# genjax-community/genjax

Hardware: AMD Instinct MI355X
Metric: particle_steps_per_sec (higher is better)
Workload: dtype f32; 1 GPU; gmm_c8_d16 ImportanceK: propagate+reweight+LSE, systematic resample, gather (BASELINE.json configs[1]); k_particles_per_gpu=1048576, k_particles_total=1048576, rng_stream=flat, exchange=none

## Files before the change

### genjax_amd/csrc/gjx_run.hip

```cpp
#include <hip/hip_ext.h>

#include "gjx_device.h"
#include "gjx_host.h"
#include "gjx_scan.h"
#include "gjx_tile.h"

#include <string.h>
#include <type_traits>

namespace gjx {

struct RunArgs {
  const gjx_site* sites;
  const float* tab;
  int n_sites, n_slots;
  key2 key;
  int64_t K, offset;
  float* choices;
  float* score;
  float* weight;
  float* logw;
  const float* logw_in;
  const float* sub;
  float* site_scores;
// ... 224 lines not shown
    else {
      score += lp;
      if (given) weight += lp;
    }
    if (a.site_scores && active) {
      float* ss = a.site_scores + (int64_t)j * K + i;
      *ss = inst == 0 ? lp : *ss + lp;
    }
    }
    }
    j0 += m;
  }
  float lw = weight;
  if (a.logw_in) lw += a.logw_in[ii];
  if (a.sub) lw -= a.sub[ii];
  if (active) {
    if (a.score) a.score[i] = score;
    if (a.weight) a.weight[i] = weight;
    if (a.logw) a.logw[i] = lw;
  }
  if (a.partials) {
    float bm, bsum;
    block_lse_partial<256>(lw, active, red, bm, bsum);
    if (a.lse) lse_publish_and_finish<256>(bm, bsum, a.partials, a.ticket, (int)gridDim.x, a.log_k_total, a.lse, red);
    else if (threadIdx.x == 0) a.partials[blockIdx.x] = pack_f2(bm, bsum);
  }
}

struct GmmArgs {
  const float* tab;
  int C;
  int logits_off, mu_off, sig_off;
  int r_off, r_len, y_off;
  key2 key;
  int64_t K, offset;
  float* choices;
  float* score;
  float* weight;
  float* logw;
  const float* logw_in;
  const float* sub;
  unsigned long long* partials;
  unsigned* ticket;
  float* lse;
  float log_k_total;
  const float* aux;
  double u;
  float* rows_out;
  int32_t* ancestors;
  unsigned long long* agg;
  unsigned* ctrl;
  unsigned long long* timeline;
  unsigned long long* tile_S;
  int32_t* tile_E;
};

template <int PPT>
struct VecStore;
template <>
struct VecStore<1> {
  static GJX_DEV void st(float* p, const float (&v)[1]) { *p = v[0]; }
};
template <>
struct VecStore<2> {
  static GJX_DEV void st(float* p, const float (&v)[2]) { *reinterpret_cast<float2*>(p) = make_float2(v[0], v[1]); }
};
template <>
struct VecStore<4> {
  static GJX_DEV void st(float* p, const float (&v)[4]) {
    *reinterpret_cast<float4*>(p) = make_float4(v[0], v[1], v[2], v[3]);
  }
};

typedef unsigned u32x4 __attribute__((ext_vector_type(4)));
constexpr int kAuxSc1 = 16;
GJX_DEV __amdgpu_buffer_rsrc_t buffer_of(const void* base, uint32_t bytes) {
  return __builtin_amdgcn_make_buffer_rsrc(const_cast<void*>(base), 0, (int)bytes, 0x00020000);
}
GJX_DEV void store4_sc1(__amdgpu_buffer_rsrc_t rs, uint32_t lane_off, uint32_t row_off, const float (&v)[4]) {
  const u32x4 x = {__float_as_uint(v[0]), __float_as_uint(v[1]), __float_as_uint(v[2]), __float_as_uint(v[3])};
  __builtin_amdgcn_raw_buffer_store_b128(x, rs, (int)lane_off, (int)row_off, kAuxSc1);
  asm volatile("s_nop 1");
}
GJX_DEV float load_sc1(__amdgpu_buffer_rsrc_t rs, uint32_t lane_off, uint32_t row_off) {
  return __uint_as_float(__builtin_amdgcn_raw_buffer_load_b32(rs, (int)lane_off, (int)row_off, kAuxSc1));
}
GJX_DEV int32_t load_sc1(const int32_t* p) { return __hip_atomic_load(p, __ATOMIC_RELAXED, __HIP_MEMORY_SCOPE_AGENT); }

template <int RNG, int D, int PPT, int THREADS>
__global__ __launch_bounds__(THREADS) void k_run_gmm(GmmArgs a) {
  constexpr int DS = D + 4;
  extern __shared__ __attribute__((aligned(16))) float smem[];
  const int C = a.C;
  float* s_mu = smem;
  float* s_sig = s_mu + C * DS;
  float* s_logit = s_sig + C * DS;
  float* s_race = s_logit + C;
  float* s_zlp = s_race + C;
  float* s_cdf = s_zlp + C;
  float* s_y = s_cdf + C;
  float* s_rr = s_y + D;
  float* s_misc = s_rr + D;
  const float* __restrict__ tab = a.tab;

  float* s_lsig = s_misc + 32;
  float* s_lr = s_lsig + C * DS;
  for (int t = threadIdx.x; t < C * D; t += THREADS) {
    const int c = t / D, d = t % D;
    const float sg = tab[a.sig_off + t];
    s_mu[c * DS + d] = tab[a.mu_off + t];
    s_sig[c * DS + d] = sg;
    s_lsig[c * DS + d] = fast_log(sg);
  }
  for (int t = threadIdx.x; t < D; t += THREADS) {
    const float r = tab[a.r_off + (a.r_len == 1 ? 0 : t)];
    s_y[t] = tab[a.y_off + t];
    s_rr[t] = fast_rcp(r);
    s_lr[t] = fast_log(r);
  }
  for (int t = threadIdx.x; t < C; t += THREADS) {
    const float l = tab[a.logits_off + t];
    s_logit[t] = l;
    s_race[t] = kLn2 * fast_exp(-l);
  }
  __syncthreads();
  if (threadIdx.x < 64) {
    float mx = -INFINITY;
    for (int c = threadIdx.x; c < C; c += 64) mx = fmaxf(mx, s_logit[c]);
    mx = wave_max(mx);
    float se = 0.0f;
    for (int c = threadIdx.x; c < C; c += 64) se += fast_exp(s_logit[c] - mx);
    se = wave_sum(se);
    const float lse = mx + fast_log(se);
    for (int c = threadIdx.x; c < C; c += 64) {
      float sl = 0.0f;
      for (int d = 0; d < D; ++d) sl += s_lsig[c * DS + d];
      s_zlp[c] = (s_logit[c] - lse) - sl - (float)D * kHalfLog2Pi;
    }
    if (threadIdx.x == 63) {
      float sl = 0.0f;
      for (int d = 0; d < D; ++d) sl += s_lr[d];
      s_misc[0] = -sl - (float)D * kHalfLog2Pi;
    }
    if (threadIdx.x == 0) {
      float run = 0.0f;
      for (int c = 0; c < C; ++c) { run += fast_exp(s_logit[c] - mx); s_cdf[c] = run; }
    }
  }
  __syncthreads();

  const int64_t K = a.K;
  const int64_t tile = (int64_t)THREADS * PPT;
  const int64_t ntiles = (K + tile - 1) / tile;
  const uint64_t goff = (uint64_t)a.offset;
  const key2 fkey = (RNG == GJX_RNG_FLAT && (goff >> 32)) ? threefry2x32(a.key, 0xFFFFFFFFu, (uint32_t)(goff >> 32)) : a.key;
  float tmax = -INFINITY;
  float tsum = 0.0f;
  for (int64_t tix = blockIdx.x; tix < ntiles; tix += gridDim.x) {
    const int64_t i0 = tix * tile + (int64_t)threadIdx.x * PPT;
    bool act[PPT];
    uint32_t c0[PPT];
    key2 sk1[PPT], sk2[PPT];
#pragma unroll
    for (int p = 0; p < PPT; ++p) {
      act[p] = (i0 + p) < K;
      const uint64_t gi = goff + (uint64_t)(act[p] ? i0 + p : K - 1);
// ... 44 lines not shown
        if (RNG == GJX_RNG_JAX32) {
          const key2 h0 = threefry2x32(sk2[p], 0u, (uint32_t)d0);
          b0 = h0.a ^ h0.b;
          if (d0 + 1 < D) { const key2 h1 = threefry2x32(sk2[p], 0u, (uint32_t)(d0 + 1)); b1 = h1.a ^ h1.b; }
        } else {
          const key2 h = threefry2x32(fkey, c0[p], (2u << GJX_FLAT_SITE_SHIFT) | (uint32_t)(d0 >> 1));
          b0 = h.a; b1 = h.b;
        }
        const int zo = z[p] * DS + d0;
        float n0, n1;
        if (RNG == GJX_RNG_FLAT) box_muller(b0, b1, n0, n1);
        else { n0 = normal_from_bits_fast(b0); n1 = (d0 + 1 < D) ? normal_from_bits_fast(b1) : 0.0f; }
        {
          const float x = fmaf(s_sig[zo], n0, s_mu[zo]);
          qx[p] = fmaf(n0, n0, qx[p]);
          const float zy = (s_y[d0] - x) * s_rr[d0];
          qy[p] = fmaf(zy, zy, qy[p]);
          xa[p] = x;
        }
        if (d0 + 1 < D) {
          const float x = fmaf(s_sig[zo + 1], n1, s_mu[zo + 1]);
          qx[p] = fmaf(n1, n1, qx[p]);
          const float zy = (s_y[d0 + 1] - x) * s_rr[d0 + 1];
          qy[p] = fmaf(zy, zy, qy[p]);
          xb[p] = x;
        } else xb[p] = 0.0f;
      }
      float* r0 = ch + (int64_t)(1 + d0) * K + i0;
      if (full) {
        VecStore<PPT>::st(r0, xa);
        if (d0 + 1 < D) VecStore<PPT>::st(r0 + K, xb);
      } else {
#pragma unroll
        for (int p = 0; p < PPT; ++p) if (act[p]) { r0[p] = xa[p]; if (d0 + 1 < D) r0[K + p] = xb[p]; }
      }
    }
    float sc[PPT], wt[PPT], lw[PPT];
#pragma unroll
    for (int p = 0; p < PPT; ++p) {
      wt[p] = fmaf(-0.5f, qy[p], s_misc[0]);
      sc[p] = fmaf(-0.5f, qx[p], s_zlp[z[p]]) + wt[p];
      float l = wt[p];
      const int64_t ii = act[p] ? i0 + p : K - 1;
      if (a.logw_in) l += a.logw_in[ii];
      if (a.sub) l -= a.sub[ii];
      lw[p] = l;
    }
    if (full) {
      if (a.score) VecStore<PPT>::st(a.score + i0, sc);
      if (a.weight) VecStore<PPT>::st(a.weight + i0, wt);
      if (a.logw) VecStore<PPT>::st(a.logw + i0, lw);
    } else {
#pragma unroll
      for (int p = 0; p < PPT; ++p) if (act[p]) {
        if (a.score) a.score[i0 + p] = sc[p];
        if (a.weight) a.weight[i0 + p] = wt[p];
        if (a.logw) a.logw[i0 + p] = lw[p];
      }
    }
#pragma unroll
    for (int p = 0; p < PPT; ++p) if (act[p]) {
      const float nm = fmaxf(tmax, lw[p]);
      if (nm > -INFINITY) tsum = tsum * fast_exp(tmax - nm) + fast_exp(lw[p] - nm);
      tmax = nm;
    }
  }
  if (a.partials) {
    constexpr int NW = THREADS / 64;
    float* red = s_misc + 8;
    const int lane = threadIdx.x & 63, wid = threadIdx.x >> 6;
    const float wm = wave_max(tmax);
    const float ws = wave_sum(wm > -INFINITY ? tsum * fast_exp(tmax - wm) : 0.0f);
    if (lane == 0) { red[wid] = wm; red[NW + wid] = ws; }
    __syncthreads();
    float bm = red[0];
    for (int w = 1; w < NW; ++w) bm = fmaxf(bm, red[w]);
    float bsum = 0.0f;
    for (int w = 0; w < NW; ++w) bsum += bm > -INFINITY ? red[NW + w] * fast_exp(red[w] - bm) : 0.0f;
    if (a.lse) lse_publish_and_finish<THREADS>(bm, bsum, a.partials, a.ticket, (int)gridDim.x, a.log_k_total, a.lse, red);
    else if (threadIdx.x == 0) a.partials[blockIdx.x] = pack_f2(bm, bsum);
  }
}

__host__ __device__ inline int gmm_aux_floats(int C, int D) { return C * (4 * D + 4) + 2 * C + 8; }

__global__ __launch_bounds__(256) void k_gmm_prepare(GmmArgs a, int D, float* aux) {
  const int C = a.C, RS = 4 * D + 4;
  const float* __restrict__ tab = a.tab;
  float* s_t = aux; float* s_zlp = s_t + C * RS; float* s_cdf = s_zlp + C; float* s_misc = s_cdf + C;
  for (int t = threadIdx.x; t < C * (D + 1); t += 256) {
    const int c = t / (D + 1), d = t % (D + 1);
    float mu = 0.0f, sg = 0.0f, av = 0.0f, bv = 0.0f;
    if (d < D) {
      mu = tab[a.mu_off + c * D + d];
      sg = tab[a.sig_off + c * D + d];
      const float rr = fast_rcp(tab[a.r_off + (a.r_len == 1 ? 0 : d)]);
      av = (tab[a.y_off + d] - mu) * rr;
      bv = sg * rr;
    }
    float* q = s_t + c * RS + 4 * d;
    q[0] = mu; q[1] = sg; q[2] = av; q[3] = bv;
  }
  if (threadIdx.x < 64) {
    float mx = -INFINITY;
    for (int c = threadIdx.x; c < C; c += 64) mx = fmaxf(mx, tab[a.logits_off + c]);
    mx = wave_max(mx);
    float se = 0.0f;
    for (int c = threadIdx.x; c < C; c += 64) se += fast_exp(tab[a.logits_off + c] - mx);
    se = wave_sum(se);
    const float lse = mx + fast_log(se);
    for (int c = threadIdx.x; c < C; c += 64) {
      float sl = 0.0f;
      for (int d = 0; d < D; ++d) sl += fast_log(tab[a.sig_off + c * D + d]);
      s_zlp[c] = (tab[a.logits_off + c] - lse) - sl - (float)D * kHalfLog2Pi;
    }
    if (threadIdx.x == 63) {
      float sl = 0.0f;
      for (int d = 0; d < D; ++d) sl += fast_log(tab[a.r_off + (a.r_len == 1 ? 0 : d)]);
      s_misc[0] = -sl - (float)D * kHalfLog2Pi;
      for (int j = 1; j < 8; ++j) s_misc[j] = 0.0f;
    }
    if (threadIdx.x == 0) {
      float run = 0.0f;
      for (int c = 0; c < C; ++c) { run += fast_exp(tab[a.logits_off + c] - mx); s_cdf[c] = run; }
    }
  }
}

template <int D, int PPT, int THREADS, bool STEP = false, bool TILES = false>
__global__ __launch_bounds__(THREADS) void k_run_gmm_flat(GmmArgs a) {
  static_assert(!STEP || (PPT == 4 && THREADS == 256), "the one-launch step works on tiles of 256 x 4 particles");
  static_assert(!TILES || (PPT == 4 && THREADS == 256 && !STEP), "tile totals: a block's tile is one quantisation tile of 1024 particles");
  __shared__ float red_tm[4];
  __shared__ uint64_t red_tq[4];
  constexpr int RS = 4 * D + 4;
  constexpr int NPAIR = (D + 1) / 2;
  unsigned epoch = 0;
  unsigned long long tag = 0;
  if (STEP && a.timeline && threadIdx.x == 0) a.timeline[blockIdx.x * 8] = __builtin_amdgcn_s_memrealtime();
  if (STEP) tag = grid_tag(a.ctrl, &epoch);
  const __amdgpu_buffer_rsrc_t rs_ch = buffer_of(a.choices, STEP ? (uint32_t)((1 + D) * a.K * 4) : 0u);
  constexpr int NHASH = (9 + 23 * (D == 1 ? 2 : D) + 63) / 64;
  constexpr bool UNROLLED = D <= 16;
  extern __shared__ __attribute__((aligned(16))) float smem[];
  const int C = a.C;
  float* s_t = smem; float* s_zlp = s_t + C * RS; float* s_cdf = s_zlp + C; float* s_misc = s_cdf + C;
  const int64_t K = a.K;
  const int64_t tile = (int64_t)THREADS * PPT;
  const int64_t ntiles = (K + tile - 1) / tile;
  const uint64_t goff = (uint64_t)a.offset;
  const key2 fkey = (goff >> 32) ? threefry2x32(a.key, 0xFFFFFFFFu, (uint32_t)(goff >> 32)) : a.key;

  const int naux = gmm_aux_floats(C, D);
  constexpr int NPRE = 4;
  float pre[NPRE];
#pragma unroll
  for (int j = 0; j < NPRE; ++j) {
    const int t = threadIdx.x + j * THREADS;
    pre[j] = t < naux ? a.aux[t] : 0.0f;
  }
  int64_t tix = blockIdx.x;
  uint32_t hz[PPT];
  auto cat_bits = [&](int64_t t) {
#pragma unroll
    for (int p = 0; p < PPT; ++p) {
      int64_t i = t * tile + (int64_t)threadIdx.x * PPT + p;
      i = i < K ? i : K - 1;
      hz[p] = threefry2x32(fkey, (uint32_t)(goff + (uint64_t)i), (1u << GJX_FLAT_SITE_SHIFT)).a;
    }
  };
  if (tix < ntiles) cat_bits(tix);
#pragma unroll
  for (int j = 0; j < NPRE; ++j) {
    const int t = threadIdx.x + j * THREADS;
    if (t < naux) smem[t] = pre[j];
  }
  for (int t = threadIdx.x + NPRE * THREADS; t < naux; t += THREADS) smem[t] = a.aux[t];
  __syncthreads();

  float tmax = -INFINITY;
  float tsum = 0.0f;
  float lw_tile[PPT];
#pragma unroll
  for (int p = 0; p < PPT; ++p) lw_tile[p] = -INFINITY;
  const float cdf_total = s_cdf[C - 1];
  for (; tix < ntiles; tix += gridDim.x) {
    const int64_t i0 = tix * tile + (int64_t)threadIdx.x * PPT;
    if (i0 >= K) break;
    uint32_t c0[PPT];
#pragma unroll
    for (int p = 0; p < PPT; ++p) c0[p] = (uint32_t)(goff + (uint64_t)(i0 + p));
    int z[PPT];
    float zf[PPT], target[PPT];
    uint32_t neg[PPT];
#pragma unroll
    for (int p = 0; p < PPT; ++p) {
      target[p] = (__uint_as_float(__builtin_amdgcn_alignbit(0x7Fu, hz[p], 9)) - 1.0f) * cdf_total;
      neg[p] = 0u;
    }
    for (int c = 0; c < C - 1; ++c) {
      const float cd = s_cdf[c];
#pragma unroll
      for (int p = 0; p < PPT; ++p) neg[p] += __float_as_uint(target[p] - cd) >> 31;
    }
#pragma unroll
    for (int p = 0; p < PPT; ++p) { z[p] = (C - 1) - (int)neg[p]; zf[p] = (float)z[p]; }
    float* ch = a.choices;
    if constexpr (STEP) store4_sc1(rs_ch, (uint32_t)i0 * 4u, 0u, zf); else VecStore<PPT>::st(ch + i0, zf);
    float qx[PPT], qy[PPT];
#pragma unroll
    for (int p = 0; p < PPT; ++p) { qx[p] = 0.0f; qy[p] = 0.0f; }
    uint32_t w[PPT][UNROLLED ? 2 * NHASH : 2];
    BitStreamRT<GJX_RNG_FLAT> bs[UNROLLED ? 1 : PPT];
    if (!UNROLLED) {
#pragma unroll
      for (int p = 0; p < PPT; ++p) { bs[p].key = fkey; bs[p].c0 = c0[p]; bs[p].site_hi = 2u << GJX_FLAT_SITE_SHIFT; bs[p].h0 = bs[p].h1 = 0xFFFFFFFFu; }
    }
    constexpr int UF = UNROLLED ? NPAIR : 1;
#pragma unroll UF
    for (int k = 0; k < NPAIR; ++k) {
      const int d0 = 2 * k;
      float xa[PPT], xb[PPT];
#pragma unroll
      for (int p = 0; p < PPT; ++p) {
        uint32_t wa, wb;
        if constexpr (UNROLLED) {
          const int last = D == 1 ? 1 : 2 * k + 1;
          const int need = (((23 * last) >> 5) + ((((23 * last) & 31) != 0) ? 1 : 0)) >> 1;
          const int prev_last = 2 * (k - 1) + 1;
          const int have = k == 0 ? -1 : ((((23 * prev_last) >> 5) + ((((23 * prev_last) & 31) != 0) ? 1 : 0)) >> 1);
#pragma unroll
          for (int h = 0; h < NHASH; ++h) if (h > have && h <= need) {
            const key2 hh = threefry2x32(fkey, c0[p], (2u << GJX_FLAT_SITE_SHIFT) | (uint32_t)h);
            w[p][2 * h] = hh.a; w[p][2 * h + 1] = hh.b;
          }
          wa = GJX_FIELD(w[p], 2 * k);
          wb = GJX_FIELD(w[p], 2 * k + 1);
        } else {
          wa = bs[p].get((uint32_t)d0);
          wb = bs[p].get((uint32_t)d0 + 1u);
        }
        const float u1 = 2.0f - __uint_as_float(__builtin_amdgcn_alignbit(0x7Fu, wa, 9));
        const float rsq = __builtin_amdgcn_logf(u1) * (-2.0f * kLn2);
        const float r = fast_sqrt(rsq);
        const float4* row = reinterpret_cast<const float4*>(s_t + z[p] * RS) + d0;
        if (D == 1) {
          const float u2 = __uint_as_float(__builtin_amdgcn_alignbit(0x7Fu, wb, 9));
          const float n0 = r * __builtin_amdgcn_cosf(u2);
          const float4 t0 = row[0];
          const float x = fmaf(t0.y, n0, t0.x);
          qx[p] = fmaf(n0, n0, qx[p]);
          const float zy = fmaf(-t0.w, n0, t0.z);
          qy[p] = fmaf(zy, zy, qy[p]);
          xa[p] = x; xb[p] = 0.0f;
        } else {
          const float u2 = __uint_as_float(__builtin_amdgcn_alignbit(0x7Fu, wb, 9));
          const float n0 = r * __builtin_amdgcn_cosf(u2), n1 = r * __builtin_amdgcn_sinf(u2);
          const float4 t0 = row[0], t1 = row[1];
          xa[p] = fmaf(t0.y, n0, t0.x);
          xb[p] = fmaf(t1.y, n1, t1.x);
          qx[p] += rsq;
          const float zy0 = fmaf(-t0.w, n0, t0.z), zy1 = fmaf(-t1.w, n1, t1.z);
          qy[p] = fmaf(zy0, zy0, qy[p]);
          qy[p] = fmaf(zy1, zy1, qy[p]);
        }
      }
      float* r0 = ch + (int64_t)(1 + d0) * K + i0;
      if constexpr (STEP) {
        store4_sc1(rs_ch, (uint32_t)i0 * 4u, (uint32_t)(1 + d0) * (uint32_t)K * 4u, xa);
        if (D > 1) store4_sc1(rs_ch, (uint32_t)i0 * 4u, (uint32_t)(2 + d0) * (uint32_t)K * 4u, xb);
      }
      else { VecStore<PPT>::st(r0, xa); if (D > 1) VecStore<PPT>::st(r0 + K, xb); }
#pragma unroll
      for (int p = 0; p < PPT; ++p) asm volatile("" : "+v"(qx[p]), "+v"(qy[p]));
      __builtin_amdgcn_sched_barrier(0);
    }
    float sc[PPT], wt[PPT], lw[PPT];
    const float wconst = s_misc[0];
#pragma unroll
    for (int p = 0; p < PPT; ++p) {
      wt[p] = fmaf(-0.5f, qy[p], wconst);
      sc[p] = fmaf(-0.5f, qx[p], s_zlp[z[p]]) + wt[p];
      float l = wt[p];
      if (a.logw_in) l += a.logw_in[i0 + p];
      if (a.sub) l -= a.sub[i0 + p];
      lw[p] = l;
    }
    if (a.score) VecStore<PPT>::st(a.score + i0, sc);
    if (a.weight) VecStore<PPT>::st(a.weight + i0, wt);
    if (a.logw) VecStore<PPT>::st(a.logw + i0, lw);
    if (STEP) {
#pragma unroll
      for (int p = 0; p < PPT; ++p) lw_tile[p] = lw[p];
    }
    float m4 = tmax;
#pragma unroll
    for (int p = 0; p < PPT; ++p) m4 = fmaxf(m4, lw[p]);
    if (m4 > -INFINITY) {
      float s4 = tsum * fast_exp(tmax - m4);
#pragma unroll
      for (int p = 0; p < PPT; ++p) s4 += fast_exp(lw[p] - m4);
      tsum = s4;
    }
    tmax = m4;
    if constexpr (TILES) {
      uint64_t q[PPT], inc;
      const int e = tile_quantise<THREADS, PPT>(lw, red_tm, red_tq, q, inc);
      if (threadIdx.x == 0) {
        const uint64_t tot = sum_partials<THREADS / 64>(red_tq);
        a.tile_S[tix] = tot;
        a.tile_E[tix] = tot ? e : kTileDead;
      }
    }
    if (tix + gridDim.x < ntiles) cat_bits(tix + gridDim.x);
  }
  constexpr int NW = THREADS / 64;
  __shared__ float red[2 * NW + 2];
  float bm = -INFINITY, bsum = 0.0f;
  if (a.partials || STEP) {
    const int lane = threadIdx.x & 63, wid = threadIdx.x >> 6;
    const float wm = wave_max(tmax);
    const float ws = wave_sum(wm > -INFINITY ? tsum * fast_exp(tmax - wm) : 0.0f);
    if (lane == 0) { red[wid] = wm; red[NW + wid] = ws; }
    __syncthreads();
    bm = red[0];
    for (int w2 = 1; w2 < NW; ++w2) bm = fmaxf(bm, red[w2]);
    for (int w2 = 0; w2 < NW; ++w2) bsum += bm > -INFINITY ? red[NW + w2] * fast_exp(red[w2] - bm) : 0.0f;
  }
  if constexpr (!STEP) {
    if (a.partials) {
      if (a.lse) lse_publish_and_finish<THREADS>(bm, bsum, a.partials, a.ticket, (int)gridDim.x, a.log_k_total, a.lse, red);
      else if (threadIdx.x == 0) a.partials[blockIdx.x] = pack_f2(bm, bsum);
    }
  } else {
    __shared__ ScanSmem sm;
#define GJX_STAMP(n) do { if (a.timeline && threadIdx.x == 0) a.timeline[blockIdx.x * 8 + (n)] = __builtin_amdgcn_s_memrealtime(); } while (0)
    GJX_STAMP(1);
    unsigned long long* aggA0 = a.agg;
    unsigned long long* aggA1 = aggA0 + gridDim.x;
    unsigned long long* aggB = aggA1 + gridDim.x;
    unsigned long long* aggC = aggB + gridDim.x;
    const int64_t i0 = (int64_t)blockIdx.x * tile + (int64_t)threadIdx.x * PPT;
    if (threadIdx.x == 0) {
      grid_publish(aggA0, tag, (unsigned long long)__float_as_uint(bm));
      grid_publish(aggA1, tag, (unsigned long long)__float_as_uint(bsum));
    }
    float gmax = -INFINITY, gsum = 0.0f;
    {
      float pm[8];
      int np = 0;
      grid_gather(aggA0, tag, a.ctrl, [&](int, unsigned long long v) { pm[np++] = __uint_as_float((uint32_t)v); });
      np = 0;
      grid_gather(aggA1, tag, a.ctrl, [&](int, unsigned long long v) {
        const float px = pm[np++], py = __uint_as_float((uint32_t)v);
        const float nm = fmaxf(gmax, px);
        if (nm > -INFINITY) gsum = gsum * fast_exp(gmax - nm) + py * fast_exp(px - nm);
        gmax = nm;
      });
    }
    {
      const float wm = wave_max(gmax);
      const float ws = wave_sum(wm > -INFINITY ? gsum * fast_exp(gmax - wm) : 0.0f);
      __syncthreads();
      if ((threadIdx.x & 63) == 0) { red[threadIdx.x >> 6] = wm; red[NW + (threadIdx.x >> 6)] = ws; }
      __syncthreads();
      gmax = fmaxf(fmaxf(red[0], red[1]), fmaxf(red[2], red[3]));
      gsum = 0.0f;
      for (int w2 = 0; w2 < 4; ++w2) gsum += gmax > -INFINITY ? red[NW + w2] * fast_exp(red[w2] - gmax) : 0.0f;
    }
    if (a.lse && blockIdx.x == 0 && threadIdx.x == 0) {
      const float l = gmax > -INFINITY ? gmax + logf(gsum) : -INFINITY;
      a.lse[0] = gmax; a.lse[1] = gsum; a.lse[2] = l; a.lse[3] = l - a.log_k_total;
    }
    GJX_STAMP(2);
    tile_scan_expand<PPT, true>(lw_tile, 1, gmax, i0, K, a.u, K, a.ancestors, nullptr, nullptr, aggB, tag, a.ctrl, epoch, false, sm);
    GJX_STAMP(3);
    asm volatile("s_waitcnt vmcnt(0)" ::: "memory");
    __syncthreads();
    if (threadIdx.x == 0) grid_publish(aggC, tag, 1ull);
    grid_gather(aggC, tag, a.ctrl, [&](int, unsigned long long) {});
    __syncthreads();
    if (blockIdx.x == 0 && threadIdx.x == 0)
      __hip_atomic_store(&a.ctrl[0], epoch + 1u, __ATOMIC_RELAXED, __HIP_MEMORY_SCOPE_AGENT);
    GJX_STAMP(4);
    int32_t an[PPT];
#pragma unroll
    for (int p = 0; p < PPT; ++p) an[p] = load_sc1(a.ancestors + i0 + p);
    constexpr int R = 1 + D;
#pragma unroll 4
    for (int r = 0; r < R; ++r) {
      float v[PPT];
#pragma unroll
      for (int p = 0; p < PPT; ++p) v[p] = load_sc1(rs_ch, (uint32_t)an[p] * 4u, (uint32_t)r * (uint32_t)K * 4u);
      VecStore<PPT>::st(a.rows_out + (int64_t)r * K + i0, v);
    }
    asm volatile("s_waitcnt vmcnt(0)" ::: "memory");
    GJX_STAMP(5);
#undef GJX_STAMP
  }
}

__global__ __launch_bounds__(256) void k_lse_finish(const float2* partials, int n, float log_k_total, float* out) {
  __shared__ float red[8];
  float m = -INFINITY;
  for (int t = threadIdx.x; t < n; t += 256) m = fmaxf(m, partials[t].x);
  m = wave_max(m);
  if ((threadIdx.x & 63) == 0) red[threadIdx.x >> 6] = m;
  __syncthreads();
  const float bm = fmaxf(fmaxf(red[0], red[1]), fmaxf(red[2], red[3]));
  float s = 0.0f;
  for (int t = threadIdx.x; t < n; t += 256) {
    const float2 p = partials[t];
    if (p.x > -INFINITY) s += p.y * fast_exp(p.x - bm);
  }
  s = wave_sum(s);
  if ((threadIdx.x & 63) == 0) red[4 + (threadIdx.x >> 6)] = s;
  __syncthreads();
  if (threadIdx.x == 0) {
    const float bs = red[4] + red[5] + red[6] + red[7];
    const float lse = bm > -INFINITY ? bm + logf(bs) : -INFINITY;
    out[0] = bm; out[1] = bs; out[2] = lse; out[3] = lse - log_k_total;
  }
}

__global__ __launch_bounds__(256) void k_lse_partial(const float* x, int64_t K, float2* partials) {
// ... 99 lines not shown
void fill_gmm_args(GmmArgs& a, const gjx_program* prog, const GmmShape& g) {
  a.tab = prog->tab_dev; a.C = g.C;
  a.logits_off = g.logits_off; a.mu_off = g.mu_off; a.sig_off = g.sig_off;
  a.r_off = g.r_off; a.r_len = g.r_len; a.y_off = g.y_off;
  a.aux = prog->aux_dev;
}

bool gmm_usable(const gjx_program* p, GmmShape* g) {
  if (env_int("GJX_FORCE_GENERIC", 0) || !match_gmm(p, g)) return false;
  if (p->rng_mode == GJX_RNG_JAX32) return true;
  return p->aux_dev != nullptr && p->n_aux >= gmm_aux_floats(g->C, g->D);
}

}

int gjx_launch_lse_finish(const void* partials, int n, int64_t K_total, float* out, hipStream_t st) {
  hipLaunchKernelGGL(k_lse_finish, dim3(1), dim3(256), 0, st, (const float2*)partials, n,
                     (float)log((double)K_total), out);
  GJX_CHECK_LAUNCH("lse_finish");
  return GJX_OK;
}

extern "C" int gjx_event_create(void** ev) {
  if (!ev) return gjx_fail(GJX_EINVAL, "gjx_event_create: bad argument");
  hipEvent_t e;
  const hipError_t r = hipEventCreate(&e);
  if (r != hipSuccess) return gjx_fail_hip(r, "gjx_event_create");
  *ev = (void*)e;
  return GJX_OK;
}
extern "C" int gjx_event_destroy(void* ev) {
  if (ev) (void)hipEventDestroy((hipEvent_t)ev);
  return GJX_OK;
}
extern "C" int gjx_event_elapsed_us(void* start, void* stop, float* us) {
  if (!start || !stop || !us) return gjx_fail(GJX_EINVAL, "gjx_event_elapsed_us: bad argument");
  hipError_t r = hipEventSynchronize((hipEvent_t)stop);
  if (r != hipSuccess) return gjx_fail_hip(r, "gjx_event_elapsed_us");
  float ms = 0.0f;
  r = hipEventElapsedTime(&ms, (hipEvent_t)start, (hipEvent_t)stop);
  if (r != hipSuccess) return gjx_fail_hip(r, "gjx_event_elapsed_us");
  *us = ms * 1000.0f;
  return GJX_OK;
}


extern "C" int gjx_program_aux_floats(const gjx_program* prog) {
  if (!prog || !prog->sites) return GJX_EINVAL;
  GmmShape g;
  if (prog->rng_mode == GJX_RNG_FLAT && match_gmm(prog, &g)) return gmm_aux_floats(g.C, g.D);
  return 0;
}

extern "C" int gjx_program_prepare(const gjx_program* prog, float* aux_dev, int32_t n_aux, void* stream) {
  if (!prog || !prog->sites || !prog->tab_dev) return gjx_fail(GJX_EINVAL, "gjx_program_prepare: null program");
  const int need = gjx_program_aux_floats(prog);
  if (need <= 0) return GJX_OK;
  if (!aux_dev || n_aux < need) return gjx_fail(GJX_EINVAL, "gjx_program_prepare: aux buffer too small (gjx_program_aux_floats)");
  GmmShape g;
  match_gmm(prog, &g);
  GmmArgs a = {};
  fill_gmm_args(a, prog, g);
  hipLaunchKernelGGL(k_gmm_prepare, dim3(1), dim3(256), 0, (hipStream_t)stream, a, g.D, aux_dev);
  GJX_CHECK_LAUNCH("gjx_program_prepare");
  return GJX_OK;
}

struct EnginePlan {
  int engine, ppt, grid;
  GmmShape g;
};

static EnginePlan plan_engine(const gjx_program* prog, int64_t K, int64_t particle_offset, bool want_site_scores, bool want_tiles = false) {
  EnginePlan e;
  e.engine = ENGINE_GENERIC; e.ppt = 1; e.grid = (int)((K + 255) / 256);
  const char* env = getenv("GJX_ENGINE");
  const bool interp = env_int("GJX_FORCE_GENERIC", 0) || (env && !strcmp(env, "interp"));
  if (interp) return e;
  const bool gen_first = env && !strcmp(env, "gen");
  const bool same_hi = ((uint64_t)particle_offset >> 32) == ((uint64_t)(particle_offset + K - 1) >> 32);
  bool has_proposal = false;
  for (int j = 0; j < prog->n_sites; ++j) has_proposal = has_proposal || (prog->sites[j].flags & GJX_SITE_PROPOSAL) || prog->sites[j].mode == GJX_MODE_OBS_PROPOSED;
  auto try_gmm = [&]() {
    if (has_proposal || want_site_scores || !same_hi || !gmm_usable(prog, &e.g)) return false;
    int ppt = env_int("GJX_GMM_PPT", 4);
    if (ppt != 1 && ppt != 2 && ppt != 4) ppt = 4;
    if (K % ppt != 0) ppt = 1;
    const int64_t tile = 256 * (int64_t)ppt, ntiles = (K + tile - 1) / tile;
    const int maxgrid = env_int("GJX_GMM_GRID", 2048);
    e.engine = ENGINE_GMM; e.ppt = ppt; e.grid = (int)(ntiles < maxgrid ? ntiles : maxgrid);
    return true;
  };
  auto try_gen = [&]() {
    if (env_int("GJX_NO_CODEGEN", 0) || !same_hi) return false;
    const int ppt = gen_pick_ppt(prog, K, want_tiles && K % 1024 == 0);
    RunVariant gv;
    if (!decode(ppt, &gv) || gen_available(prog, ppt) != GJX_OK) return false;
    const int64_t tile = gv.particles_per_block(), ntiles = (K + tile - 1) / tile;
    static const int resident = [] { int dev = 0, cus = 256; (void)hipGetDevice(&dev); (void)hipDeviceGetAttribute(&cus, hipDeviceAttributeMultiprocessorCount, dev); return 4 * (cus > 0 ? cus : 256); }();
    int maxgrid = env_int("GJX_GEN_GRID", gv.mfma ? (1 << 20) : (gv.wide ? 2 * resident : resident));
    if (gv.wide && maxgrid > (int)((K + 255) / 256) && maxgrid > 4096) maxgrid = (int)((K + 255) / 256) > 4096 ? (int)((K + 255) / 256) : 4096;
    e.engine = ENGINE_GEN; e.ppt = ppt; e.grid = (int)(ntiles < maxgrid ? ntiles : maxgrid);
    return true;
  };
  if (gen_first) { if (!try_gen()) try_gmm(); }
  else if (!try_gmm()) try_gen();
  return e;
}

extern "C" int gjx_program_engine(const gjx_program* prog) {
  if (!prog || !prog->sites) return GJX_EINVAL;
  return plan_engine(prog, 1024, 0, false).engine;
}

extern "C" int gjx_run_partials_count(const gjx_program* prog, int64_t K, int64_t particle_offset) {
  if (!prog || !prog->sites || K <= 0) return GJX_EINVAL;
  return plan_engine(prog, K, particle_offset, false).grid;
}

extern "C" int gjx_run_program(const gjx_program* prog, uint32_t key0, uint32_t key1, int64_t K,
                               int64_t particle_offset, float* choices, float* score, float* weight,
                               float* logw, const float* logw_in, const float* sub,
                               float* site_scores, float* lse, int64_t K_total, void* workspace,
                               size_t workspace_bytes, void* stream) {
  gjx_run_opts o;
  memset(&o, 0, sizeof(o));
  return gjx_run_program_ex(prog, key0, key1, K, particle_offset, choices, score, weight, logw, logw_in, sub, site_scores, lse, K_total,
                            workspace, workspace_bytes, stream, &o, nullptr);
}

extern "C" int gjx_run_program_ex(const gjx_program* prog, uint32_t key0, uint32_t key1, int64_t K,
                                  int64_t particle_offset, float* choices, float* score, float* weight,
                                  float* logw, const float* logw_in, const float* sub,
                                  float* site_scores, float* lse, int64_t K_total, void* workspace,
                                  size_t workspace_bytes, void* stream, const gjx_run_opts* opts, gjx_run_info* info_out) {
  gjx_run_opts no_opts;
  memset(&no_opts, 0, sizeof(no_opts));
  const gjx_run_opts& op = opts ? *opts : no_opts;
  gjx_run_info info = {0, 0, 0};
  hipEvent_t ev0 = nullptr, ev1 = nullptr;
  if (op.flags & GJX_RUN_TIME_DISPATCH) { ev0 = (hipEvent_t)op.start_event; ev1 = (hipEvent_t)op.stop_event; }
  if (info_out) *info_out = info;
  if (!prog || !prog->sites || !prog->sites_dev || !prog->tab_dev) return gjx_fail(GJX_EINVAL, "gjx_run_program: null program");
  if (K < 0 || prog->n_sites < 0) return gjx_fail(GJX_EINVAL, "gjx_run_program: negative size");
  if (K == 0) return GJX_OK;
  if (prog->n_slots > 0 && !choices) return gjx_fail(GJX_EINVAL, "gjx_run_program: choices is null");
  if (lse && !logw) return gjx_fail(GJX_EINVAL, "gjx_run_program: lse needs logw");
  if (prog->rng_mode == GJX_RNG_FLAT) {
    int plain = 0, local = 0, tag = 0;
    for (int j = 0; j < prog->n_sites; ++j) {
      const int sc = prog->sites[j].scan;
      if (sc == 0) { ++plain; tag = 0; }
      else { if (sc != tag) { tag = sc; local = 0; } ++local; }
      if (plain > GJX_FLAT_MAX_SITES || local > GJX_FLAT_MAX_SITES)
        return gjx_fail(GJX_EUNSUPPORTED, "gjx_run_program: FLAT stream supports at most 1023 sites per Scan step and 1023 outside Scans");
    }
  }
  for (int j = 0; j < prog->n_sites; ++j) {
    const gjx_site& sj = prog->sites[j];
    if (sj.mode != GJX_MODE_OBS_MASK) continue;
    if (sj.kind == GJX_DIRICHLET) return gjx_fail(GJX_EUNSUPPORTED, "gjx_run_program: a dirichlet site cannot be masked per particle");
    if (sj.slot < 0 || sj.obs_off < 0 || sj.obs_off >= prog->n_slots) return gjx_fail(GJX_EINVAL, "gjx_run_program: OBS_MASK needs a value slot and a flag slot");
  }
  hipStream_t st = (hipStream_t)stream;
  unsigned long long* partials = nullptr;
  unsigned* ticket = nullptr;
  if (lse || (workspace && logw)) {
// ... 179 lines not shown
```

Measured before the change: 18.72 billion particle-steps/s.

## Use 32-bit indexing, buffer loads/stores, and popcount CDF search in flat GMM kernel

Converts the flat GMM kernel's particle indexing from 64-bit to 32-bit arithmetic, capping K on the host so the narrower math stays valid. Global loads and stores of choices, scores, weights and aux go through per-tile buffer resources. The categorical CDF search packs comparison sign bits 32 at a time and counts them with popcount. The aim is to cut address arithmetic and per-comparison ALU work. The cost is more per-tile descriptor setup and reliance on buffer-descriptor bounds behaviour.

```diff
diff --git a/genjax_amd/csrc/gjx_run.hip b/genjax_amd/csrc/gjx_run.hip
--- a/genjax_amd/csrc/gjx_run.hip
+++ b/genjax_amd/csrc/gjx_run.hip
@@ -330,6 +330,45 @@
   __builtin_amdgcn_raw_buffer_store_b128(x, rs, (int)lane_off, (int)row_off, kAuxSc1);
   asm volatile("s_nop 1");
 }
+template <int PPT>
+struct BufStore;
+template <>
+struct BufStore<1> {
+  static GJX_DEV void st(__amdgpu_buffer_rsrc_t rs, uint32_t lane_off, const float (&v)[1]) {
+    __builtin_amdgcn_raw_buffer_store_b32(__float_as_uint(v[0]), rs, (int)lane_off, 0, 0);
+  }
+};
+template <>
+struct BufStore<2> {
+  static GJX_DEV void st(__amdgpu_buffer_rsrc_t rs, uint32_t lane_off, const float (&v)[2]) {
+    typedef unsigned u32x2 __attribute__((ext_vector_type(2)));
+    const u32x2 x = {__float_as_uint(v[0]), __float_as_uint(v[1])};
+    __builtin_amdgcn_raw_buffer_store_b64(x, rs, (int)lane_off, 0, 0);
+  }
+};
+template <>
+struct BufStore<4> {
+  static GJX_DEV void st(__amdgpu_buffer_rsrc_t rs, uint32_t lane_off, const float (&v)[4]) {
+    const u32x4 x = {__float_as_uint(v[0]), __float_as_uint(v[1]), __float_as_uint(v[2]), __float_as_uint(v[3])};
+    __builtin_amdgcn_raw_buffer_store_b128(x, rs, (int)lane_off, 0, 0);
+    asm volatile("s_nop 1");
+  }
+};
+GJX_DEV float buf_load1(__amdgpu_buffer_rsrc_t rs, uint32_t lane_off) {
+  return __uint_as_float(__builtin_amdgcn_raw_buffer_load_b32(rs, (int)lane_off, 0, 0));
+}
+template <int PPT>
+GJX_DEV void buf_load(__amdgpu_buffer_rsrc_t rs, uint32_t lane_off, float (&v)[PPT]) {
+  static_assert(PPT == 1 || PPT == 2 || PPT == 4, "one load of 4, 8 or 16 bytes per lane");
+  if constexpr (PPT == 1) v[0] = buf_load1(rs, lane_off);
+  else if constexpr (PPT == 2) {
+    const auto x = __builtin_amdgcn_raw_buffer_load_b64(rs, (int)lane_off, 0, 0);
+    v[0] = __uint_as_float(x[0]); v[1] = __uint_as_float(x[1]);
+  } else {
+    const auto x = __builtin_amdgcn_raw_buffer_load_b128(rs, (int)lane_off, 0, 0);
+    v[0] = __uint_as_float(x[0]); v[1] = __uint_as_float(x[1]); v[2] = __uint_as_float(x[2]); v[3] = __uint_as_float(x[3]);
+  }
+}
 GJX_DEV float load_sc1(__amdgpu_buffer_rsrc_t rs, uint32_t lane_off, uint32_t row_off) {
   return __uint_as_float(__builtin_amdgcn_raw_buffer_load_b32(rs, (int)lane_off, (int)row_off, kAuxSc1));
 }
@@ -540,6 +579,7 @@
   }
 }
 
+constexpr int64_t kGmmMaxK = 0xFFFFF000ll;
 __host__ __device__ inline int gmm_aux_floats(int C, int D) { return C * (4 * D + 4) + 2 * C + 8; }
 
 __global__ __launch_bounds__(256) void k_gmm_prepare(GmmArgs a, int D, float* aux) {
@@ -597,35 +637,32 @@
   unsigned long long tag = 0;
   if (STEP && a.timeline && threadIdx.x == 0) a.timeline[blockIdx.x * 8] = __builtin_amdgcn_s_memrealtime();
   if (STEP) tag = grid_tag(a.ctrl, &epoch);
-  const __amdgpu_buffer_rsrc_t rs_ch = buffer_of(a.choices, STEP ? (uint32_t)((1 + D) * a.K * 4) : 0u);
+  __amdgpu_buffer_rsrc_t rs_ch;
+  if constexpr (STEP) rs_ch = buffer_of(a.choices, (uint32_t)((1 + D) * a.K * 4));
   constexpr int NHASH = (9 + 23 * (D == 1 ? 2 : D) + 63) / 64;
   constexpr bool UNROLLED = D <= 16;
   extern __shared__ __attribute__((aligned(16))) float smem[];
   const int C = a.C;
   float* s_t = smem; float* s_zlp = s_t + C * RS; float* s_cdf = s_zlp + C; float* s_misc = s_cdf + C;
-  const int64_t K = a.K;
-  const int64_t tile = (int64_t)THREADS * PPT;
-  const int64_t ntiles = (K + tile - 1) / tile;
+  const uint32_t K = (uint32_t)a.K;
+  constexpr uint32_t tile = (uint32_t)THREADS * PPT;
+  const uint32_t ntiles = K / tile + (K % tile != 0u);
   const uint64_t goff = (uint64_t)a.offset;
+  const uint32_t lane0 = threadIdx.x * PPT;
   const key2 fkey = (goff >> 32) ? threefry2x32(a.key, 0xFFFFFFFFu, (uint32_t)(goff >> 32)) : a.key;
 
   const int naux = gmm_aux_floats(C, D);
+  const __amdgpu_buffer_rsrc_t rs_aux = buffer_of(a.aux, (uint32_t)naux * 4u);
   constexpr int NPRE = 4;
   float pre[NPRE];
 #pragma unroll
-  for (int j = 0; j < NPRE; ++j) {
-    const int t = threadIdx.x + j * THREADS;
-    pre[j] = t < naux ? a.aux[t] : 0.0f;
-  }
-  int64_t tix = blockIdx.x;
+  for (int j = 0; j < NPRE; ++j) pre[j] = buf_load1(rs_aux, (threadIdx.x + j * THREADS) * 4u);
+  uint32_t tix = blockIdx.x;
   uint32_t hz[PPT];
-  auto cat_bits = [&](int64_t t) {
-#pragma unroll
-    for (int p = 0; p < PPT; ++p) {
-      int64_t i = t * tile + (int64_t)threadIdx.x * PPT + p;
-      i = i < K ? i : K - 1;
-      hz[p] = threefry2x32(fkey, (uint32_t)(goff + (uint64_t)i), (1u << GJX_FLAT_SITE_SHIFT)).a;
-    }
+  auto cat_bits = [&](uint32_t t) {
+#pragma unroll
+    for (int p = 0; p < PPT; ++p)
+      hz[p] = threefry2x32(fkey, (uint32_t)goff + (t * tile + lane0 + (uint32_t)p), (1u << GJX_FLAT_SITE_SHIFT)).a;
   };
   if (tix < ntiles) cat_bits(tix);
 #pragma unroll
@@ -633,7 +670,8 @@
     const int t = threadIdx.x + j * THREADS;
     if (t < naux) smem[t] = pre[j];
   }
-  for (int t = threadIdx.x + NPRE * THREADS; t < naux; t += THREADS) smem[t] = a.aux[t];
+#pragma unroll 1
+  for (int t = threadIdx.x + NPRE * THREADS; t < naux; t += THREADS) smem[t] = buf_load1(rs_aux, (uint32_t)t * 4u);
   __syncthreads();
 
   float tmax = -INFINITY;
@@ -643,28 +681,43 @@
   for (int p = 0; p < PPT; ++p) lw_tile[p] = -INFINITY;
   const float cdf_total = s_cdf[C - 1];
   for (; tix < ntiles; tix += gridDim.x) {
-    const int64_t i0 = tix * tile + (int64_t)threadIdx.x * PPT;
+    const uint32_t t0 = tix * tile;
+    const uint32_t i0 = t0 + lane0;
     if (i0 >= K) break;
+    const uint32_t tile_bytes = (K - t0 < tile ? K - t0 : tile) * 4u;
+    const uint32_t lane_off = lane0 * 4u;
+    auto put = [&](float* base, uint32_t row, const float (&v)[PPT]) {
+      if constexpr (STEP) store4_sc1(rs_ch, i0 * 4u, row * K * 4u, v);
+      else BufStore<PPT>::st(buffer_of(base + ((uint64_t)row * K + t0), tile_bytes), lane_off, v);
+    };
     uint32_t c0[PPT];
 #pragma unroll
-    for (int p = 0; p < PPT; ++p) c0[p] = (uint32_t)(goff + (uint64_t)(i0 + p));
+    for (int p = 0; p < PPT; ++p) c0[p] = (uint32_t)goff + (i0 + (uint32_t)p);
     int z[PPT];
     float zf[PPT], target[PPT];
     uint32_t neg[PPT];
 #pragma unroll
     for (int p = 0; p < PPT; ++p) {
       target[p] = (__uint_as_float(__builtin_amdgcn_alignbit(0x7Fu, hz[p], 9)) - 1.0f) * cdf_total;
+      asm volatile("" : "+v"(target[p]));
       neg[p] = 0u;
     }
-    for (int c = 0; c < C - 1; ++c) {
-      const float cd = s_cdf[c];
-#pragma unroll
-      for (int p = 0; p < PPT; ++p) neg[p] += __float_as_uint(target[p] - cd) >> 31;
+    for (int cb = 0; cb < C - 1; cb += 32) {
+      const int ce = cb + 32 < C - 1 ? cb + 32 : C - 1;
+      uint32_t sg[PPT];
+#pragma unroll
+      for (int p = 0; p < PPT; ++p) sg[p] = 0u;
+      for (int c = cb; c < ce; ++c) {
+        const float cd = s_cdf[c];
+#pragma unroll
+        for (int p = 0; p < PPT; ++p) sg[p] = __builtin_amdgcn_alignbit(sg[p], __float_as_uint(target[p] - cd), 31);
+      }
+#pragma unroll
+      for (int p = 0; p < PPT; ++p) neg[p] += (uint32_t)__builtin_popcount(sg[p]);
     }
 #pragma unroll
     for (int p = 0; p < PPT; ++p) { z[p] = (C - 1) - (int)neg[p]; zf[p] = (float)z[p]; }
-    float* ch = a.choices;
-    if constexpr (STEP) store4_sc1(rs_ch, (uint32_t)i0 * 4u, 0u, zf); else VecStore<PPT>::st(ch + i0, zf);
+    put(a.choices, 0u, zf);
     float qx[PPT], qy[PPT];
 #pragma unroll
     for (int p = 0; p < PPT; ++p) { qx[p] = 0.0f; qy[p] = 0.0f; }
@@ -701,7 +754,7 @@
         const float u1 = 2.0f - __uint_as_float(__builtin_amdgcn_alignbit(0x7Fu, wa, 9));
         const float rsq = __builtin_amdgcn_logf(u1) * (-2.0f * kLn2);
         const float r = fast_sqrt(rsq);
-        const float4* row = reinterpret_cast<const float4*>(s_t + z[p] * RS) + d0;
+        const float4* row = reinterpret_cast<const float4*>(s_t + __umul24((uint32_t)z[p], (uint32_t)RS)) + d0;
         if (D == 1) {
           const float u2 = __uint_as_float(__builtin_amdgcn_alignbit(0x7Fu, wb, 9));
           const float n0 = r * __builtin_amdgcn_cosf(u2);
@@ -722,31 +775,37 @@
           qy[p] = fmaf(zy0, zy0, qy[p]);
           qy[p] = fmaf(zy1, zy1, qy[p]);
         }
-      }
-      float* r0 = ch + (int64_t)(1 + d0) * K + i0;
-      if constexpr (STEP) {
-        store4_sc1(rs_ch, (uint32_t)i0 * 4u, (uint32_t)(1 + d0) * (uint32_t)K * 4u, xa);
-        if (D > 1) store4_sc1(rs_ch, (uint32_t)i0 * 4u, (uint32_t)(2 + d0) * (uint32_t)K * 4u, xb);
-      }
-      else { VecStore<PPT>::st(r0, xa); if (D > 1) VecStore<PPT>::st(r0 + K, xb); }
+        if (D > 1) asm volatile("" : "+v"(xa[p]), "+v"(xb[p])); else asm volatile("" : "+v"(xa[p]));
+      }
+      put(a.choices, (uint32_t)(1 + d0), xa);
+      if (D > 1) put(a.choices, (uint32_t)(2 + d0), xb);
 #pragma unroll
       for (int p = 0; p < PPT; ++p) asm volatile("" : "+v"(qx[p]), "+v"(qy[p]));
       __builtin_amdgcn_sched_barrier(0);
     }
-    float sc[PPT], wt[PPT], lw[PPT];
+    float sc[PPT], wt[PPT], lw[PPT], lin[PPT], lsub[PPT];
     const float wconst = s_misc[0];
+    if (a.logw_in) buf_load<PPT>(buffer_of(a.logw_in + t0, tile_bytes), lane_off, lin);
+    if (a.sub) buf_load<PPT>(buffer_of(a.sub + t0, tile_bytes), lane_off, lsub);
 #pragma unroll
     for (int p = 0; p < PPT; ++p) {
       wt[p] = fmaf(-0.5f, qy[p], wconst);
       sc[p] = fmaf(-0.5f, qx[p], s_zlp[z[p]]) + wt[p];
+      asm volatile("" : "+v"(wt[p]), "+v"(sc[p]));
       float l = wt[p];
-      if (a.logw_in) l += a.logw_in[i0 + p];
-      if (a.sub) l -= a.sub[i0 + p];
+      if (a.logw_in) l += lin[p];
+      if (a.sub) l -= lsub[p];
       lw[p] = l;
     }
-    if (a.score) VecStore<PPT>::st(a.score + i0, sc);
-    if (a.weight) VecStore<PPT>::st(a.weight + i0, wt);
-    if (a.logw) VecStore<PPT>::st(a.logw + i0, lw);
+    if constexpr (STEP) {
+      if (a.score) VecStore<PPT>::st(a.score + i0, sc);
+      if (a.weight) VecStore<PPT>::st(a.weight + i0, wt);
+      if (a.logw) VecStore<PPT>::st(a.logw + i0, lw);
+    } else {
+      if (a.score) put(a.score, 0u, sc);
+      if (a.weight) put(a.weight, 0u, wt);
+      if (a.logw) put(a.logw, 0u, lw);
+    }
     if (STEP) {
 #pragma unroll
       for (int p = 0; p < PPT; ++p) lw_tile[p] = lw[p];
@@ -799,6 +858,7 @@
     unsigned long long* aggB = aggA1 + gridDim.x;
     unsigned long long* aggC = aggB + gridDim.x;
     const int64_t i0 = (int64_t)blockIdx.x * tile + (int64_t)threadIdx.x * PPT;
+    const int64_t K = a.K;
     if (threadIdx.x == 0) {
       grid_publish(aggA0, tag, (unsigned long long)__float_as_uint(bm));
       grid_publish(aggA1, tag, (unsigned long long)__float_as_uint(bsum));
@@ -1064,7 +1124,7 @@
   bool has_proposal = false;
   for (int j = 0; j < prog->n_sites; ++j) has_proposal = has_proposal || (prog->sites[j].flags & GJX_SITE_PROPOSAL) || prog->sites[j].mode == GJX_MODE_OBS_PROPOSED;
   auto try_gmm = [&]() {
-    if (has_proposal || want_site_scores || !same_hi || !gmm_usable(prog, &e.g)) return false;
+    if (has_proposal || want_site_scores || !same_hi || K > kGmmMaxK || !gmm_usable(prog, &e.g)) return false;
     int ppt = env_int("GJX_GMM_PPT", 4);
     if (ppt != 1 && ppt != 2 && ppt != 4) ppt = 4;
     if (K % ppt != 0) ppt = 1;
```

Measured after the change: 18.67 billion particle-steps/s. Within noise of the previous version (-0.2%).
